# rvp-group/srrg2_laser_slam_2d

Measured on AMD Instinct MI355X. Metric: scan-to-map alignments/sec (1081-beam vs 100k-pt map, 20 GN iters), higher is better.
Workload: dtype f32

## Files before the change

### srrg2_laser_slam_2d_amd/csrc/lsm2d_device_cand.h

```cpp
LSM2D_DEV float cand_depth_margin(float r, float m_t, float tn2 ) { return m_t + __builtin_fmaf(1.0e-6f, r, __builtin_fmaf(2.6e-7f, tn2, 1e-7f)); }
LSM2D_DEV int cand_classify_polar(const ProjK& P, float r, float th, float u, int col , float m_t, float m_th, float tn2, float& md) {
  md = cand_depth_margin(r, m_t, tn2);
  if (r < P.rmin - md || r > P.rmax + md) return 0;
  if (!(md <= 0.25f * r)) return 1;
  const float aK = __builtin_fabsf(P.K00);
  const float cs = __builtin_fmaf(aK, __builtin_fmaf(1.06f, md / (r - md), 1.001f * m_th), 4e-3f);
  if ((3.14159274101257324f - __builtin_fabsf(th)) * aK <= cs) return 1;
  if (u < -cs || u > P.colsf + cs) return 0;
  if ((unsigned) col >= (unsigned) P.cols) return 1;
  if (!(r >= P.rmin + md && r <= P.rmax - md)) return 1;
  const float f = u - (float) col;
  return (f > cs && 1.0f - f > cs) ? 2 : 1;
}
template <bool kGuarded>
LSM2D_DEV int cand_classify(const Iso& T, const ProjK& P, float px, float py, float m_t, float m_th, float tn2, float& r, float& md, int& col) {
  r = 0.0f; md = 0.0f; col = -1;
  if (!(__builtin_fabsf(px) < __builtin_huge_valf() && __builtin_fabsf(py) < __builtin_huge_valf())) return 0;
  float qx, qy;
  xf_point(T, px, py, qx, qy);
  const float r2 = __builtin_fmaf(qx, qx, qy * qy);
  if (!(r2 >= 1e-30f && r2 <= 1e37f)) return 1;
  float y0;
  r = sqrt_rn_seed(r2, y0);
  const float th = bearing<kGuarded>(qy, qx, r, y0);
  const float u = __builtin_fmaf(P.K00, th, P.K01);
  asm("v_cvt_flr_i32_f32 %0, %1" : "=v"(col) : "v"(u));
  const int cl = cand_classify_polar(P, r, th, u, col, m_t, m_th, tn2, md);
  if ((unsigned) col >= (unsigned) P.cols) col = -1;
  return cl;
}
template <bool kGuarded>
LSM2D_DEV void project_point_stream_blk(const Iso& T, const ProjK& P, float px, float py, int idx, u64* canvas, uint32_t* blk, const int* par) {
  float qx, qy;
  xf_point(T, px, py, qx, qy);
  const float r2 = __builtin_fmaf(qx, qx, qy * qy);
  if (r2 >= P.r2lo && r2 <= P.r2hi) {
    float y0;
    const float r  = sqrt_rn_seed(r2, y0);
    const float th = bearing<kGuarded>(qy, qx, r, y0);
    const float u  = __builtin_fmaf(P.K00, th, P.K01);
    int col;
    asm("v_cvt_flr_i32_f32 %0, %1" : "=v"(col) : "v"(u));
    if ((unsigned) col < (unsigned) P.cols) {
      atomicMin(&canvas[col], ((u64) __float_as_uint(r) << 32) | (u64) (uint32_t) idx);
      const float m_t = __int_as_float(par[4]), m_th = __int_as_float(par[5]);
      const float tn2 = __builtin_fabsf(T.tx) + __builtin_fabsf(T.ty) + 2.0f * m_t;
      float md;
      if (cand_classify_polar(P, r, th, u, col, m_t, m_th, tn2, md) == 2) atomicMin(&blk[col], __float_as_uint(r + md));
    }
  }
}
template <bool kGuarded, int kStride>
LSM2D_DEV void project_cloud_list_blk_t(const float4* __restrict__ lane_xy, int T_steps, const Iso& Tin, const ProjK& Pin, u64* canvas, int tid, int nthreads,
                                        const uint16_t* units, int n_units, int B, uint32_t* blk, const int* par) {
  const Iso T = Tin; ProjK P = Pin;
  asm volatile("" : "+v"(P.K01));
  typedef unsigned u32x4 __attribute__((ext_vector_type(4)));
  const unsigned long long pb = reinterpret_cast<unsigned long long>(lane_xy);
  const unsigned pb_hi = (unsigned) __builtin_amdgcn_readfirstlane((int) (pb >> 32));
  const unsigned pb_lo = (unsigned) __builtin_amdgcn_readfirstlane((int) (unsigned) pb);
  float4* ubase = reinterpret_cast<float4*>(((unsigned long long) pb_hi << 32) | (unsigned long long) pb_lo);
  const __amdgpu_buffer_rsrc_t rsrc = __builtin_amdgcn_make_buffer_rsrc(ubase, (short) 0, 0x7fffffff, 0x00020000);
  const int row_bytes = nthreads * (int) sizeof(float4);
  for (int k = tid; k < n_units; k += kStride) {
    const int code = (int) units[k];
    const int g = code & 511, t0 = (code >> 9) * B;
    const int nsteps = T_steps - t0 < B ? T_steps - t0 : B;
    const int voff = g * (int) sizeof(float4) + t0 * row_bytes;
    int idx = 2 * (g * T_steps + t0);
    auto load = [&](int soff) {
      const u32x4 w = __builtin_amdgcn_raw_buffer_load_b128(rsrc, voff, soff, 0);
      return make_float4(__uint_as_float(w.x), __uint_as_float(w.y), __uint_as_float(w.z), __uint_as_float(w.w));
    };
    auto pair = [&](const float4& v, int i) {
      project_point_stream_blk<kGuarded>(T, P, v.x, v.y, i, canvas, blk, par);
      project_point_stream_blk<kGuarded>(T, P, v.z, v.w, i + 1, canvas, blk, par);
    };
    int t = 0, soff = 0;
    float4 va = load(0);
    for (; t + 2 <= nsteps; t += 2) {
      const float4 vb = load(soff + row_bytes);
      pair(va, idx);
      soff += 2 * row_bytes;
      va = load(soff);
      pair(vb, idx + 2);
      idx += 4;
    }
    if (t < nsteps) pair(va, idx);
  }
}
template <int kStride, class F>
LSM2D_DEV void cand_for_each_pair(const float4* __restrict__ lane_xy, int T_steps, int tid, int nthreads, const uint16_t* units, int n_units, int B, F f) {
  typedef unsigned u32x4 __attribute__((ext_vector_type(4)));
  const unsigned long long pb = reinterpret_cast<unsigned long long>(lane_xy);
  const unsigned pb_hi = (unsigned) __builtin_amdgcn_readfirstlane((int) (pb >> 32));
  const unsigned pb_lo = (unsigned) __builtin_amdgcn_readfirstlane((int) (unsigned) pb);
  float4* ubase = reinterpret_cast<float4*>(((unsigned long long) pb_hi << 32) | (unsigned long long) pb_lo);
  const __amdgpu_buffer_rsrc_t rsrc = __builtin_amdgcn_make_buffer_rsrc(ubase, (short) 0, 0x7fffffff, 0x00020000);
  const int row_bytes = nthreads * (int) sizeof(float4);
  for (int k = tid; k < n_units; k += kStride) {
    const int code = (int) units[k];
    const int g = code & 511, t0 = (code >> 9) * B;
    const int nsteps = T_steps - t0 < B ? T_steps - t0 : B;
    const int voff = g * (int) sizeof(float4) + t0 * row_bytes;
    int idx = 2 * (g * T_steps + t0);
    for (int t = 0; t < nsteps; ++t, idx += 2) {
      const u32x4 w = __builtin_amdgcn_raw_buffer_load_b128(rsrc, voff + t * row_bytes, 0, 0);
      f(__uint_as_float(w.x), __uint_as_float(w.y), __uint_as_float(w.z), __uint_as_float(w.w), idx);
    }
  }
}
template <bool kGuarded, int kStride>
LSM2D_DEV void cand_collect_t(const float4* __restrict__ lane_xy, int T_steps, const Iso& Tin, const ProjK& Pin, int tid, int nthreads, const uint16_t* units, int n_units, int B,
                              const uint32_t* blk, uint32_t* cand, int cap, int* count, float m_t, float m_th) {
  const Iso T = Tin; const ProjK P = Pin;
  const float tn2 = __builtin_fabsf(T.tx) + __builtin_fabsf(T.ty) + 2.0f * m_t;
  auto keeps = [&](float px, float py) -> bool {
    float r, md; int col;
    const int cl = cand_classify<kGuarded>(T, P, px, py, m_t, m_th, tn2, r, md, col);
    if (cl != 2) return cl == 1;
    return !(__uint_as_float(blk[col]) < r - md);
  };
  cand_for_each_pair<kStride>(lane_xy, T_steps, tid, nthreads, units, n_units, B, [&](float ax, float ay, float bx, float by, int idx) {
    const bool k0 = keeps(ax, ay), k1 = keeps(bx, by);
    const u64 b0 = __ballot(k0), b1 = __ballot(k1);
    const u64 act = b0 | b1;
    if (act) {
      const int n0 = __popcll(b0);
      int base = 0;
      if ((int) __builtin_amdgcn_mbcnt_hi((unsigned) (act >> 32), __builtin_amdgcn_mbcnt_lo((unsigned) act, 0u)) == 0 && (k0 || k1)) base = atomicAdd(count, n0 + __popcll(b1));
      base = __builtin_amdgcn_readlane(base, __builtin_amdgcn_readfirstlane(__builtin_ctzll(act)));
      const int p0 = base + (int) __builtin_amdgcn_mbcnt_hi((unsigned) (b0 >> 32), __builtin_amdgcn_mbcnt_lo((unsigned) b0, 0u));
      const int p1 = base + n0 + (int) __builtin_amdgcn_mbcnt_hi((unsigned) (b1 >> 32), __builtin_amdgcn_mbcnt_lo((unsigned) b1, 0u));
      if (k0 && p0 < cap) cand[p0] = (uint32_t) idx;
      if (k1 && p1 < cap) cand[p1] = (uint32_t) (idx + 1);
    }
  });
}
template <bool kGuarded, int kStride>
LSM2D_DEV void project_candidates_t(const float2* __restrict__ mxy, const Iso& Tin, const ProjK& Pin, u64* canvas, int tid, const uint32_t* cand, int n) {
  const Iso T = Tin; ProjK P = Pin;
  asm volatile("" : "+v"(P.K01));
  int k = tid;
  if (k >= n) return;
  int idx = (int) cand[k];
  float2 p = mxy[idx];
  for (; k < n; k += kStride) {
    const int kn = k + kStride;
    const int idn = (int) cand[kn < n ? kn : k];
    const float2 pn = mxy[idn];
    project_point_stream<kGuarded>(T, P, p.x, p.y, idx, canvas);
    idx = idn; p = pn;
  }
}
LSM2D_HD int cand_blocker_words(int cols) { return (cols + 3) & ~3; }
template <int kStride>
LSM2D_DEV void cand_clear_blockers(const ProjK& P, int tid, uint32_t* blk) { for (int c = tid; c < P.cols; c += kStride) blk[c] = 0xFFFFFFFFu; }
template <int kStride>
LSM2D_DEV void project_cloud_list_blk(const float4* __restrict__ lane_xy, int T_steps, const Iso& T, const ProjK& P, u64* canvas, int tid, int nthreads,
                                      const uint16_t* units, int n_units, int B, uint32_t* blk, const int* par) {
  if (P.tiny_ok) project_cloud_list_blk_t<false, kStride>(lane_xy, T_steps, T, P, canvas, tid, nthreads, units, n_units, B, blk, par);
  else project_cloud_list_blk_t<true, kStride>(lane_xy, T_steps, T, P, canvas, tid, nthreads, units, n_units, B, blk, par);
}
template <int kStride, int kChunks>
LSM2D_DEV void cand_collect(const float4* lane_xy, int T_steps, const Iso& T, const ProjK& P, int tid, const uint16_t* units, int n_units, int B, uint32_t* blk, const int* par, int* count) {
  const int cap = __builtin_amdgcn_readfirstlane(par[1]);
  const float m_t = __int_as_float(__builtin_amdgcn_readfirstlane(par[4])), m_th = __int_as_float(__builtin_amdgcn_readfirstlane(par[5]));
  uint32_t* cand = blk + cand_blocker_words(P.cols);
  if (P.tiny_ok) cand_collect_t<false, kStride>(lane_xy, T_steps, T, P, tid, kChunks, units, n_units, B, blk, cand, cap, count, m_t, m_th);
  else cand_collect_t<true, kStride>(lane_xy, T_steps, T, P, tid, kChunks, units, n_units, B, blk, cand, cap, count, m_t, m_th);
}
LSM2D_DEV bool cand_pose_within(const Iso& N, const Iso& L, float m_t, float m_th) {
  if (__float_as_uint(N.c) == __float_as_uint(L.c) && __float_as_uint(N.s) == __float_as_uint(L.s)) {
    const float ex = N.tx - L.tx, ey = N.ty - L.ty;
    return ex * ex + ey * ey <= m_t * m_t * 0.999999f;
  }
  const float cd = N.c * L.c + N.s * L.s, sd = N.s * L.c - N.c * L.s;
  const float dx = N.tx - (cd * L.tx - sd * L.ty), dy = N.ty - (sd * L.tx + cd * L.ty);
  const float lim = m_t - 4e-7f * (__builtin_fabsf(N.tx) + __builtin_fabsf(N.ty) + __builtin_fabsf(L.tx) + __builtin_fabsf(L.ty));
  return cd > 0.5f && __builtin_fabsf(sd) <= m_th - 3e-7f && lim > 0.0f && dx * dx + dy * dy <= lim * lim * 0.999999f;
}
```

Baseline: 2.317 million.

## Batch candidate compaction per 16-step segment with wave prefix sum

Candidate collection now makes each lane accumulate a keep bitmask over a segment of up to 16 steps. The wave then does one prefix-sum compaction and one atomicAdd per segment, instead of a ballot and atomic per step pair. The unit loop becomes wave-uniform so lanes iterate in lockstep, and the loads are software-pipelined two at a time. The block-depth lookup is made branchless. This cuts atomics and cross-lane operations, but writes become per-lane scattered runs and idle lanes pay for the segment loop.

```diff
diff --git a/srrg2_laser_slam_2d_amd/csrc/lsm2d_device_cand.h b/srrg2_laser_slam_2d_amd/csrc/lsm2d_device_cand.h
--- a/srrg2_laser_slam_2d_amd/csrc/lsm2d_device_cand.h
+++ b/srrg2_laser_slam_2d_amd/csrc/lsm2d_device_cand.h
@@ -89,8 +89,9 @@
     if (t < nsteps) pair(va, idx);
   }
 }
-template <int kStride, class F>
-LSM2D_DEV void cand_for_each_pair(const float4* __restrict__ lane_xy, int T_steps, int tid, int nthreads, const uint16_t* units, int n_units, int B, F f) {
+static constexpr int kCandSegSteps = 16;
+template <int kStride, class F, class E>
+LSM2D_DEV void cand_for_each_pair(const float4* __restrict__ lane_xy, int T_steps, int tid, int nthreads, const uint16_t* units, int n_units, int B, F f, E end) {
   typedef unsigned u32x4 __attribute__((ext_vector_type(4)));
   const unsigned long long pb = reinterpret_cast<unsigned long long>(lane_xy);
   const unsigned pb_hi = (unsigned) __builtin_amdgcn_readfirstlane((int) (pb >> 32));
@@ -98,43 +99,57 @@
   float4* ubase = reinterpret_cast<float4*>(((unsigned long long) pb_hi << 32) | (unsigned long long) pb_lo);
   const __amdgpu_buffer_rsrc_t rsrc = __builtin_amdgcn_make_buffer_rsrc(ubase, (short) 0, 0x7fffffff, 0x00020000);
   const int row_bytes = nthreads * (int) sizeof(float4);
-  for (int k = tid; k < n_units; k += kStride) {
-    const int code = (int) units[k];
+  const int lane = tid & 63;
+  for (int kw = __builtin_amdgcn_readfirstlane(tid - lane); kw < n_units; kw += kStride) {
+    const bool have = kw + lane < n_units;
+    const int code = have ? (int) units[kw + lane] : 0;
     const int g = code & 511, t0 = (code >> 9) * B;
-    const int nsteps = T_steps - t0 < B ? T_steps - t0 : B;
-    const int voff = g * (int) sizeof(float4) + t0 * row_bytes;
-    int idx = 2 * (g * T_steps + t0);
-    for (int t = 0; t < nsteps; ++t, idx += 2) {
-      const u32x4 w = __builtin_amdgcn_raw_buffer_load_b128(rsrc, voff + t * row_bytes, 0, 0);
-      f(__uint_as_float(w.x), __uint_as_float(w.y), __uint_as_float(w.z), __uint_as_float(w.w), idx);
+    const int usteps = !have ? 0 : T_steps - t0 < B ? T_steps - t0 : B;
+    for (int s0 = 0; s0 < B; s0 += kCandSegSteps) {
+      const int nsteps = usteps - s0 < kCandSegSteps ? usteps - s0 : kCandSegSteps;
+      const int voff = nsteps > 0 ? g * (int) sizeof(float4) + (t0 + s0) * row_bytes : 0;
+      auto load = [&](int soff) { return __builtin_amdgcn_raw_buffer_load_b128(rsrc, voff, soff, 0); };
+      auto pair = [&](const u32x4& w, int t) { f(__uint_as_float(w.x), __uint_as_float(w.y), __uint_as_float(w.z), __uint_as_float(w.w), t); };
+      int t = 0, soff = 0;
+      u32x4 va = load(0);
+      for (; t + 2 <= nsteps; t += 2) {
+        const u32x4 vb = load(soff + row_bytes);
+        pair(va, t);
+        soff += 2 * row_bytes;
+        va = load(soff);
+        pair(vb, t + 1);
+      }
+      if (t < nsteps) pair(va, t);
+      end(2 * (g * T_steps + t0 + s0));
     }
   }
 }
+LSM2D_DEV int wave_sum63_i(int v);
 template <bool kGuarded, int kStride>
 LSM2D_DEV void cand_collect_t(const float4* __restrict__ lane_xy, int T_steps, const Iso& Tin, const ProjK& Pin, int tid, int nthreads, const uint16_t* units, int n_units, int B,
                               const uint32_t* blk, uint32_t* cand, int cap, int* count, float m_t, float m_th) {
   const Iso T = Tin; const ProjK P = Pin;
   const float tn2 = __builtin_fabsf(T.tx) + __builtin_fabsf(T.ty) + 2.0f * m_t;
-  auto keeps = [&](float px, float py) -> bool {
-    float r, md; int col;
-    const int cl = cand_classify<kGuarded>(T, P, px, py, m_t, m_th, tn2, r, md, col);
-    if (cl != 2) return cl == 1;
-    return !(__uint_as_float(blk[col]) < r - md);
-  };
-  cand_for_each_pair<kStride>(lane_xy, T_steps, tid, nthreads, units, n_units, B, [&](float ax, float ay, float bx, float by, int idx) {
-    const bool k0 = keeps(ax, ay), k1 = keeps(bx, by);
-    const u64 b0 = __ballot(k0), b1 = __ballot(k1);
-    const u64 act = b0 | b1;
-    if (act) {
-      const int n0 = __popcll(b0);
+  unsigned mask = 0;
+  cand_for_each_pair<kStride>(lane_xy, T_steps, tid, nthreads, units, n_units, B, [&](float ax, float ay, float bx, float by, int t) {
+    float r0, md0, r1, md1; int col0, col1;
+    const int cl0 = cand_classify<kGuarded>(T, P, ax, ay, m_t, m_th, tn2, r0, md0, col0);
+    const int cl1 = cand_classify<kGuarded>(T, P, bx, by, m_t, m_th, tn2, r1, md1, col1);
+    const float b0 = __uint_as_float(blk[cl0 == 2 ? col0 : 0]), b1 = __uint_as_float(blk[cl1 == 2 ? col1 : 0]);
+    const bool k0 = cl0 == 2 ? !(b0 < r0 - md0) : cl0 == 1, k1 = cl1 == 2 ? !(b1 < r1 - md1) : cl1 == 1;
+    mask |= ((k0 ? 1u : 0u) | (k1 ? 2u : 0u)) << (2 * t);
+  }, [&](int idx0) {
+    const int n = __popc(mask);
+    const int incl = wave_sum63_i(n);
+    const int total = __builtin_amdgcn_readlane(incl, 63);
+    if (total) {
       int base = 0;
-      if ((int) __builtin_amdgcn_mbcnt_hi((unsigned) (act >> 32), __builtin_amdgcn_mbcnt_lo((unsigned) act, 0u)) == 0 && (k0 || k1)) base = atomicAdd(count, n0 + __popcll(b1));
-      base = __builtin_amdgcn_readlane(base, __builtin_amdgcn_readfirstlane(__builtin_ctzll(act)));
-      const int p0 = base + (int) __builtin_amdgcn_mbcnt_hi((unsigned) (b0 >> 32), __builtin_amdgcn_mbcnt_lo((unsigned) b0, 0u));
-      const int p1 = base + n0 + (int) __builtin_amdgcn_mbcnt_hi((unsigned) (b1 >> 32), __builtin_amdgcn_mbcnt_lo((unsigned) b1, 0u));
-      if (k0 && p0 < cap) cand[p0] = (uint32_t) idx;
-      if (k1 && p1 < cap) cand[p1] = (uint32_t) (idx + 1);
+      if ((tid & 63) == 0) base = atomicAdd(count, total);
+      int pos = __builtin_amdgcn_readfirstlane(base) + incl - n;
+      for (unsigned m = mask; m; m &= m - 1, ++pos)
+        if (pos < cap) cand[pos] = (uint32_t) (idx0 + __builtin_ctz(m));
     }
+    mask = 0;
   });
 }
 template <bool kGuarded, int kStride>
```

Measured after the change: 2.383 million (median of 6 runs). 1.03x the previous value.
